# jtdaugherty/flux

Measured on AMD Instinct MI355X. Metric: Msamples/sec on demo2.yml (fixed spp), higher is better.
Workload: dtype f64

## Files before the change

### flux_amd/csrc/abi.hip

```cpp
#include <hip/hip_runtime.h>

#include <chrono>
#include <cmath>
#include <cstdarg>
#include <cstdio>
#include <cstring>
#include <memory>
#include <new>
#include <algorithm>
#include <cstdlib>
#include <string>
#include <vector>

#include "../../include/flux_abi.h"
#include "flux_device.h"
#include "flux_tables.h"
#include "flux_math_coeffs.h"

#include "flux_ctx.h"

namespace flux {

thread_local std::string g_last_error;

// ... 42 lines not shown
    hipError_t e = hipMemcpy(d, xy, sizeof(xy), hipMemcpyHostToDevice);
    if (e == hipSuccess) e = flux::generate_sampler_grid(FLUX_SAMPLER_REGULAR, 0, 2, d, nullptr, nullptr);
    if (e == hipSuccess) e = hipStreamCreateWithFlags(&s, hipStreamNonBlocking);
    if (s) (void)hipStreamDestroy(s);
    (void)hipFree(d);
    if (e != hipSuccess) return fail(FLUX_E_DEVICE, "flux_device_warmup: %s", hipGetErrorString(e));
    return FLUX_OK;
}

static void free_ctx(flux_ctx *c) {
    if (!c) return;
    DeviceGuard g(c->device);
    if (c->ev0) (void)hipEventDestroy(c->ev0);
    if (c->ev1) (void)hipEventDestroy(c->ev1);
    (void)hipFree(c->d_shapes);
    (void)hipFree(c->d_mats);
    (void)hipFree(c->d_fscene);
    (void)hipFree(c->d_pix);
    (void)hipFree(c->d_disc);
    (void)hipFree(c->d_hemi);
    (void)hipFree(c->d_gloss);
    (void)hipFree(c->d_glossx);
    (void)hipFree(c->d_gxoff);
    (void)hipFree(c->d_setrows);
    (void)hipFree(c->d_rowperm);
    (void)hipFree(c->d_invperm);
    (void)hipFree(c->d_stats);
    (void)hipFree(c->d_tris);
    (void)hipFree(c->d_nodes);
    (void)hipFree(c->d_nodesq);
    (void)hipFree(c->d_arena);
    (void)hipFree(c->d_out);
    delete c;
}

void flux_ctx_destroy(flux_ctx *ctx) { free_ctx(ctx); }

}

namespace flux {

static int validate_material(const flux_material &m, const char *what, uint64_t i) {
    if (m.kind < FLUX_MAT_MATTE || m.kind > FLUX_MAT_DIELECTRIC)
        return fail(FLUX_E_INVALID, "%s %llu: unknown material kind %d", what, (unsigned long long)i, m.kind);
    if (m.kind == FLUX_MAT_DIELECTRIC && !(std::isfinite(m.k) && m.k > 0.0))
        return fail(FLUX_E_INVALID, "%s %llu: dielectric refraction index must be finite and > 0, got %g", what, (unsigned long long)i, m.k);
// ... 103 lines not shown
    };
    auto copy = [&](void *dst, const auto &v) {
        if (e == hipSuccess) e = hipMemcpy(dst, v.data(), v.size() * sizeof(v[0]), hipMemcpyHostToDevice);
    };
    auto alloc_copy = [&](auto **p, const auto &v) {
        alloc(p, v.size() * sizeof(v[0]));
        copy(*p, v);
    };
    alloc_copy(&c->d_shapes, h.shapes);
    alloc(&c->d_mats, h.mats.size() * sizeof(DevMaterial) + h.wtab.size() * sizeof(double));
    copy(c->d_mats, h.mats);
    copy(c->d_mats + h.mats.size(), h.wtab);
    alloc_copy(&c->d_fscene, h.fscene);
    alloc(&c->d_pix, pix_bytes);
    alloc(&c->d_disc, pix_bytes);
    alloc(&c->d_hemi, hemi_bytes);
    alloc(&c->d_gloss, pix_bytes * 2);
    const char *tables_env = std::getenv("FLUX_SAMPLE_TABLES");
    const int gx_stride = (tables_env && std::atoi(tables_env) == 0) ? 0 : h.rp.gx_stride;
    if (gx_stride) {
        alloc(&c->d_glossx, own * c->N * (size_t)gx_stride);
        alloc_copy(&c->d_gxoff, h.gx_off);
    }
    alloc(&c->d_setrows, own * sizeof(DevSetRows));
    alloc(&c->d_rowperm, perm_bytes);
    alloc(&c->d_invperm, perm_bytes);
    alloc(&c->d_stats, FLUX_NUM_STATS * sizeof(unsigned long long));
    if (!h.tris.empty()) {
        alloc_copy(&c->d_tris, h.tris);
        alloc_copy(&c->d_nodes, h.nodes);
        alloc_copy(&c->d_nodesq, h.nodesq);
        if (!h.arena.empty()) alloc_copy(&c->d_arena, h.arena);
    }
    if (e == hipSuccess) e = hipMemset(c->d_stats, 0, FLUX_NUM_STATS * sizeof(unsigned long long));
    laps.lap(FLUX_CREATE_MS_UPLOAD);
    if (e == hipSuccess) e = hipEventCreate(&c->ev0);
    if (e == hipSuccess) e = hipEventCreate(&c->ev1);
    laps.lap(FLUX_CREATE_MS_OTHER);
    double tab_ms[3] = {0, 0, 0};
    if (e == hipSuccess)
        e = generate_tables(seed, c->S, c->sets, c->D, c->n, c->H, c->d_pix, c->d_disc, c->d_hemi, c->d_rowperm, c->d_invperm, nullptr, tab_ms);
    if (e == hipSuccess) {
        e = generate_gloss_table(c->d_pix, (size_t)c->sets.count * c->N, c->d_gloss, nullptr);
        if (e == hipSuccess && gx_stride)
            e = generate_glossx_table(c->d_gloss, (size_t)c->sets.count * c->N, h.gx_inv_e1.data(), h.rp.n_gloss_exp, gx_stride / 16,
                                      c->d_glossx, nullptr);
// ... 11 lines not shown
            rows[m].hemi = c->d_hemi + m * c->D * c->N * kHemiDoubles;
            rows[m].gloss = c->d_gloss + m * c->N * 4;
            rows[m].glossx = gx_stride ? c->d_glossx + m * c->N * (size_t)(gx_stride / 16) : nullptr;
        }
        copy(c->d_setrows, rows);
    }
    if (e != hipSuccess)
        return fail(e == hipErrorOutOfMemory ? FLUX_E_NOMEM : FLUX_E_DEVICE, "flux_ctx_create: %s", hipGetErrorString(e));

    RenderParams &rp = c->rp;
    rp = h.rp;
    rp.pixel_denom = 1.0 / (double)((uint64_t)c->n * c->n);
    rp.max_depth = (int32_t)c->D;
    rp.nsamp = c->N;
    rp.shapes = c->d_shapes;
    rp.mats = c->d_mats;
    rp.pix = c->d_pix;
    rp.disc = c->d_disc;
    rp.hemi = c->d_hemi;
    rp.gloss = c->d_gloss;
    rp.glossx = c->d_glossx;
    rp.gx_off = c->d_gxoff;
    rp.gx_stride = gx_stride;
    rp.set_rows = c->d_setrows;
    rp.rowperm = c->d_rowperm;
    rp.invperm = c->d_invperm;
    for (int k = 0; k < 12; k++) rp.exp2c[k] = fastmath::kExp2Poly[k];
    rp.tris = c->d_tris;
    rp.nodes = c->d_nodes;
    rp.nodesq = c->d_nodesq;
    rp.nodes4 = reinterpret_cast<const DevNode4Q *>(c->d_arena);
    const unsigned char *fs = c->d_fscene;
    rp.fsph = reinterpret_cast<const DevScanSphere *>(fs + h.fs.sph);
    rp.fpln = reinterpret_cast<const DevScanPlane *>(fs + h.fs.pln);
    rp.frec = reinterpret_cast<const DevHitRec *>(fs + h.fs.rec);
    rp.fsph32 = h.filter32 ? reinterpret_cast<const DevScanSphere32 *>(fs + h.fs.s32) : nullptr;
    rp.f32_half = rp.fsph32 && h.f32_half >= 0 ? rp.fsph32 + h.f32_half : nullptr;
    rp.f32_top = rp.fsph32 ? rp.fsph32 + h.f32_top : nullptr;
    rp.sshapes = reinterpret_cast<const DevShape *>(fs + h.fs.ss);
    rp.pxc = reinterpret_cast<const double *>(fs + h.fs.pxc);
    rp.fdsk = reinterpret_cast<const DevScanDisk *>(fs + h.fs.dsk);
    rp.fbox = reinterpret_cast<const DevScanBox *>(fs + h.fs.box);
    laps.lap(FLUX_CREATE_MS_UPLOAD);
    laps.ms[FLUX_CREATE_MS_TOTAL] = 0.0;
    for (int k = 1; k < FLUX_CREATE_TIMING_WORDS; k++) laps.ms[FLUX_CREATE_MS_TOTAL] += laps.ms[k];
    for (int k = 0; k < FLUX_CREATE_TIMING_WORDS; k++) c->create_ms[k] = laps.ms[k];
// ... 454 lines not shown
```

### flux_amd/csrc/flux_ctx.h

```cpp
#pragma once
#include <hip/hip_runtime.h>

#include <chrono>
#include <new>
#include <string>
#include <system_error>

#include "../../include/flux_abi.h"
#include "flux_device.h"
#include "flux_tables.h"
#include "scene_build.h"

namespace flux {

extern thread_local std::string g_last_error;
int fail(int code, const char *fmt, ...) __attribute__((format(printf, 2, 3)));

template <class F> int no_throw(F &&f) {
    try {
        return f();
    } catch (const std::bad_alloc &) {
        return fail(FLUX_E_NOMEM, "host allocation failed");
    } catch (const std::system_error &e) {
        return fail(FLUX_E_NOMEM, "%s", e.what());
// ... 31 lines not shown

#define HIP_TRY(expr)                                                                             \
    do {                                                                                          \
        hipError_t e_ = (expr);                                                                   \
        if (e_ != hipSuccess)                                                                     \
            return flux::fail(e_ == hipErrorOutOfMemory ? FLUX_E_NOMEM : FLUX_E_DEVICE, "%s: %s", \
                              #expr, hipGetErrorString(e_));                                      \
    } while (0)

struct flux_ctx {
    int device = 0;
    flux::RenderParams rp{};
    uint64_t seed = 0;
    uint32_t n = 0, N = 0, D = 0, S = 0, W = 0, H = 0;
    flux::SetRange sets{0, 1, 0};
    flux::DevShape *d_shapes = nullptr;
    flux::DevMaterial *d_mats = nullptr;
    unsigned char *d_fscene = nullptr;
    double2 *d_pix = nullptr, *d_disc = nullptr;
    double *d_hemi = nullptr;
    double *d_gloss = nullptr;
    double2 *d_glossx = nullptr;
    int32_t *d_gxoff = nullptr;
    flux::DevSetRows *d_setrows = nullptr;
    int32_t *d_rowperm = nullptr, *d_invperm = nullptr;
    unsigned long long *d_stats = nullptr;
    bool stats_on = false;
    flux::DevTri *d_tris = nullptr;
    flux::DevNode *d_nodes = nullptr;
    flux::DevNode4A *d_arena = nullptr;
    flux::DevNodeQ *d_nodesq = nullptr;
    flux::BvhInfo bvh{};
    int traversal = FLUX_TRAVERSE_BVH;
    int variant = FLUX_KERNEL_DEFAULT;
    int math = FLUX_MATH_FAST;
    double *d_out = nullptr;
    size_t d_out_doubles = 0;
    hipEvent_t ev0 = nullptr, ev1 = nullptr;
    bool timed = false;
    uint64_t device_bytes = 0;
    double U[3], V[3], Wv[3];
    double create_ms[FLUX_CREATE_TIMING_WORDS] = {};
};
```

### flux_amd/csrc/flux_device.h

```cpp
#pragma once
#include <hip/hip_runtime.h>
#include <stdint.h>

#include "flux_bvh.h"


#ifndef FLUX_UNI_SPHERES
#define FLUX_UNI_SPHERES 2
#endif
#ifndef FLUX_BVH_WIDE_MAX_STACK
#define FLUX_BVH_WIDE_MAX_STACK 48
#endif
#ifndef FLUX_MAX_WAVES_PER_PIXEL
#define FLUX_MAX_WAVES_PER_PIXEL 4
#endif
#ifndef FLUX_MIN_SAMPLES_PER_WAVE
#define FLUX_MIN_SAMPLES_PER_WAVE 4096
#endif

namespace flux {

constexpr int kHemiDoubles = 4;
constexpr double kTMin = 0.0005;
constexpr double kPi = 3.14159265358979323846264338327950288;
// ... 138 lines not shown
    int32_t self_skip;
    int32_t n_uni, uni_idx[2];
    int32_t unit_dirs;
    int32_t env_short, pad_env;
    double env_radius;
    double t_min, env_deep;
    double env_px, env_py, env_pz, env_rr;
    double env_eps;
    const DevScanSphere32 *f32_half, *f32_top;
    int32_t f32_groups;
    uint32_t f32_valid;
    double fwx, fwy, fwz;
    const double *pxc;
    const DevSetRows *set_rows;
    double exp2c[12];
    const DevScanDisk *fdsk;
    int32_t n_dsk;
    int32_t has_diel;
    const double2 *glossx;
    const int32_t *gx_off;
    int32_t gx_stride, n_gloss_exp;
    const DevScanBox *fbox;
    int32_t n_box;
};

__host__ __device__ inline int hit_records(const RenderParams &p) { return p.n_sph + p.n_pln + p.n_dsk + 6 * p.n_box; }

}
```

### flux_amd/csrc/flux_plan.h

```cpp
#pragma once
#include <stddef.h>
#include <stdint.h>

#include "flux_device.h"

#ifndef FLUX_BLOCK_THREADS
#define FLUX_BLOCK_THREADS 64
#endif
#ifndef FLUX_WPE_SPLIT
#define FLUX_WPE_SPLIT 5
#endif
#ifndef FLUX_HITQ_MIN_TAKE
#define FLUX_HITQ_MIN_TAKE 32
#endif

namespace flux {

constexpr int kGlossExpSlots = 4;

constexpr int kQueueDoubles = 9;
constexpr int kQueueBytesPerWave = (kQueueDoubles * 64) * 8 + 2 * 64 * 4;
constexpr int kHitQDoubles = 7;
constexpr int kHitQInts = 3;
constexpr int kHitQBytesPerSlot = kHitQDoubles * 8 + kHitQInts * 4;
constexpr uint32_t kHitQDwordsPerSlot = kHitQBytesPerSlot / 4;
constexpr uint32_t hitq_entry_dword(uint32_t C, uint32_t k) { return (C - 1u - k) * kHitQDwordsPerSlot; }
constexpr bool hitq_admits_phase_a(uint32_t C, uint32_t nhit) { return nhit + 64u <= C; }

enum KernelCopy { kCopyStrict = 0, kCopyFast = 1, kCopyFastDiel = 2 };
KernelCopy kernel_copy(const RenderParams &p, int math);

struct LaunchPlan {
    int kernel = -1;
    unsigned block = 64;
    uint64_t blocks = 0;
    size_t lds = 0;
    unsigned waves_per_pixel = 1;
    int lds_scene = 0;
    int hq_cap = 0, hq_th = 0, hq_bits = 0;
    int copy = kCopyFast;
    int tris = 0;
    int typ = 0;
    int max32 = 0;
};
LaunchPlan plan_render(const RenderParams &p, int variant, int math);

size_t lane_stacks_lds(int math, size_t depth, bool tris, size_t bvh_stack, size_t lanes);
size_t shade_rays_lds(const RenderParams &p, int math);

}
// ... 1 lines not shown
```

### flux_amd/csrc/launch_plan.cpp

```cpp
#include <algorithm>
#include <cstdlib>

#include "flux_plan.h"
#include "../../include/flux_abi.h"

namespace flux {

KernelCopy kernel_copy(const RenderParams &p, int math) {
    if (math == FLUX_MATH_STRICT) return kCopyStrict;
    return p.has_diel ? kCopyFastDiel : kCopyFast;
}

size_t lane_stacks_lds(int math, size_t depth, bool tris, size_t bvh_stack, size_t lanes) {
    return (math == FLUX_MATH_STRICT ? depth * 4 * lanes * sizeof(double) : 0) + (tris ? bvh_stack * lanes * sizeof(int) : 0);
}

size_t shade_rays_lds(const RenderParams &p, int math) {
    return lane_stacks_lds(math, (size_t)p.max_depth, p.n_tris > 0, (size_t)p.bvh_stack, 64);
}

static bool split_typ(const RenderParams &p) {
    return p.n_sph <= 32 && p.glossy_long == 0 && p.unit_dirs == 1 && p.self_skip == 1 && p.env_short == 1 && p.n_uni == 1 &&
           p.fsph32 != nullptr && p.n_dsk == 0 && p.n_box == 0 && p.has_diel == 0 && (p.n_gloss_exp == 0 || p.gx_stride != 0);
}
static bool bvh4_typ(const RenderParams &p, bool lds_scene) {
    return lds_scene && p.n_sph <= 32 && p.glossy_long == 0 && p.unit_dirs == 1 && p.self_skip == 1 && p.n_uni == 1 &&
           p.fsph32 != nullptr && p.n_dsk == 0 && p.n_box == 0 && p.has_diel == 0;
}

LaunchPlan plan_render(const RenderParams &p, int variant, int math) {
    LaunchPlan L;
    L.copy = kernel_copy(p, math);
    const bool fast = L.copy != kCopyStrict;
    const uint32_t N = p.nsamp;
    const uint64_t npix = (uint64_t)p.num_rows * (uint64_t)p.img_w;
    if (npix == 0 || p.set_count <= 0) return L;
    if (variant == FLUX_KERNEL_DEFAULT) variant = N >= 256u ? FLUX_KERNEL_SPLIT : FLUX_KERNEL_REFILL;
    if (N < 64u) variant = FLUX_KERNEL_STATIC;
    const uint32_t lpp = N >= 64u ? 64u : N;
    const uint32_t ppw = 64u / lpp;
    uint64_t waves = (npix + ppw - 1) / ppw;
    if (variant != FLUX_KERNEL_STATIC && p.num_sets == (uint32_t)p.img_w)
        waves = 8ull * ((uint64_t)(p.set_count / 8) * (uint64_t)p.num_rows +
                        ((uint64_t)(p.set_count % 8) * (uint64_t)p.num_rows + 7u) / 8u);
    unsigned K = 1;
    if (variant != FLUX_KERNEL_STATIC)
        while (K * 2u <= (unsigned)FLUX_MAX_WAVES_PER_PIXEL && (uint64_t)K * 2u * FLUX_MIN_SAMPLES_PER_WAVE <= N) K *= 2u;
    const bool tris = p.n_tris > 0;
    if (!fast && variant != FLUX_KERNEL_STATIC)
        while (K > 1u && lane_stacks_lds(math, (size_t)p.max_depth, tris, (size_t)p.bvh_stack, 64 * K) > 60 * 1024) K /= 2u;
    const unsigned block = (variant == FLUX_KERNEL_STATIC) ? FLUX_BLOCK_THREADS : 64u * K;
    const unsigned wpb = (variant == FLUX_KERNEL_STATIC) ? block / 64 : 1u;
    L.blocks = (waves + wpb - 1) / wpb;
    if (fast && variant != FLUX_KERNEL_STATIC && tris && p.bvh_stack > 0) {
        L.block = 64;
        size_t lds4 = (size_t)(p.bvh4_stack > 0 ? p.bvh4_stack : 1) * 64 * sizeof(int);
        const size_t scene4 = (size_t)hit_records(p) * sizeof(DevHitRec) + (size_t)p.n_mats * sizeof(DevMaterial) +
                              (size_t)p.n_sph * sizeof(DevScanSphere);
        const bool lds_scene4 = lds4 + scene4 <= 7680;
        if (lds_scene4) lds4 += scene4;
        if (p.nodes4 != nullptr && p.bvh4_stack <= FLUX_BVH_WIDE_MAX_STACK) {
            L.kernel = 4;
            L.lds = lds4;
            L.lds_scene = lds_scene4 ? 1 : 0;
            L.typ = bvh4_typ(p, lds_scene4) ? 1 : 0;
        } else {
            L.kernel = 3;
            L.lds = (size_t)p.bvh_stack * 64 * sizeof(int);
        }
        return L;
    }
    const size_t scene_lds = (size_t)hit_records(p) * sizeof(DevHitRec) + (size_t)p.n_sph * sizeof(DevScanSphere);
    if (fast && variant == FLUX_KERNEL_SPLIT && !tris && p.n_sph <= 64 && scene_lds <= 16384) {
        L.kernel = 2;
        L.block = block;
        L.waves_per_pixel = K;
        L.lds = (size_t)kQueueBytesPerWave * K + scene_lds;
        L.typ = split_typ(p) ? 1 : 0;
        L.max32 = p.n_sph <= 32 ? 1 : 0;
        if (p.glossy_long == 0 && p.has_diel == 0) {
            const size_t granules = (size_t)128 * K / (4 * FLUX_WPE_SPLIT);
            const size_t per_wave = granules * 1280 > scene_lds + 96 ? (granules * 1280 - scene_lds - 96) / K : 0;
            uint32_t cap = (uint32_t)(per_wave / kHitQBytesPerSlot) & ~1u;
            if (const char *e = std::getenv("FLUX_SPLIT_HITQ_CAP")) cap = std::min(cap, (uint32_t)std::max(0, std::atoi(e)) & ~1u);
            uint32_t th = cap > 64u + FLUX_HITQ_MIN_TAKE ? std::min(64u, cap - 64u) : FLUX_HITQ_MIN_TAKE;
            if (const char *e = std::getenv("FLUX_SPLIT_HITQ_TAKE_AT")) th = (uint32_t)std::max(1, std::min(64, std::atoi(e)));
            int bits = 1;
            while ((1 << bits) < hit_records(p)) ++bits;
            if (cap >= 64u + th && bits * p.max_depth <= 32) {
                L.hq_cap = (int)cap;
                L.hq_th = (int)th;
                L.hq_bits = bits;
                L.lds = (size_t)cap * kHitQBytesPerSlot * K + scene_lds;
            }
        }
        return L;
    }
    L.kernel = variant == FLUX_KERNEL_STATIC ? 0 : 1;
    L.block = block;
    L.waves_per_pixel = variant == FLUX_KERNEL_STATIC ? 1 : K;
    L.lds = lane_stacks_lds(math, (size_t)p.max_depth, tris, (size_t)p.bvh_stack, block);
    L.tris = tris ? 1 : 0;
    return L;
}

}
```

### flux_amd/csrc/render_body.inc

```

#undef FLUX_STAGE
#if FLUX_FAST
#define FLUX_STAGE() __builtin_amdgcn_sched_barrier(0)
#else
#define FLUX_STAGE() ((void)0)
#endif

struct Ray {
    double ox, oy, oz, dx, dy, dz;
};

typedef const __attribute__((address_space(4))) RenderParams *ParamsInKernarg;
static_assert(sizeof(DevMaterial) % 16 == 0, "the bounce-weight records behind the materials are read as double2");
__device__ __forceinline__ const RenderParams &relaunder_params(uint32_t tick) {
    ParamsInKernarg p = (ParamsInKernarg)__builtin_amdgcn_kernarg_segment_ptr();
    asm("" : "+s"(p) : "s"(tick));
    return *(const RenderParams *)p;
}

__device__ __forceinline__ unsigned long long ballot64(bool b) { return __builtin_amdgcn_ballot_w64(b); }
__device__ __forceinline__ bool any64(bool b) { return __builtin_amdgcn_ballot_w64(b) != 0ull; }
__device__ __forceinline__ bool all64(bool b) { return __builtin_amdgcn_ballot_w64(!b) == 0ull; }

typedef double flux_d2 __attribute__((ext_vector_type(2)));
// ... 1607 lines not shown
            const double e = fastmath::fsqrt_nonneg(__builtin_fmax(dq, 0.0));
            double t = (-hb - e) * rs;
            if (!(t > tmin)) t = (-hb + e) * rs;
            bool ok = dq >= 0.0 && t > tmin;
            if (any_zflat) {
                if (zflat && box_z_nan_miss(P, r, k)) ok = false;
            }
            if (ok) {
                bool take = best < 0 || t < tb;
                if (!take && t == tb) take = best >= P.n_sph ? P.frec[k].orig_id < best_id : k < best;
                if (take) {
                    best = k;
                    tb = t;
                }
            }
        }
    }
}

__device__ __forceinline__ double lds_dword_pair(const uint32_t *p) { return __hiloint2double((int)p[1], (int)p[0]); }
__device__ __forceinline__ void lds_dword_pair_store(uint32_t *p, double v) {
    p[0] = (uint32_t)__double2loint(v);
    p[1] = (uint32_t)__double2hiint(v);
}

template <bool STATS, bool MAX32, bool TYP, bool HQ = false>
__global__ __launch_bounds__(64 * FLUX_MAX_WAVES_PER_PIXEL, FLUX_WPE_SPLIT) void render_split_kernel(const RenderParams P0, int hq_cap, int hq_th,
                                                                                                  int hq_bits) {
    (void)hq_cap;
    (void)hq_th;
    (void)hq_bits;
    const RenderParams &P = P0;
    extern __shared__ double lds_stack[];
    __shared__ double part[FLUX_MAX_WAVES_PER_PIXEL][3];
    const int tid = threadIdx.x;
    const uint32_t lane = tid & 63;
    const uint32_t N = P.nsamp;
    const uint32_t K = blockDim.x >> 6, sub = (uint32_t)__builtin_amdgcn_readfirstlane(tid >> 6);
    const uint32_t s_lo = (uint32_t)((uint64_t)N * sub / K), s_hi = (uint32_t)((uint64_t)N * (sub + 1) / K);
    const int n_rec = TYP ? P.n_sph + P.n_pln + P.n_dsk : hit_records(P);
    const size_t scene_lds_bytes = (size_t)n_rec * sizeof(DevHitRec) + (size_t)P.n_sph * sizeof(DevScanSphere);
    double *q = lds_stack + scene_lds_bytes / 8 + (size_t)sub * (HQ ? (size_t)hq_cap * kHitQBytesPerSlot / 8 : kQueueBytesPerWave / 8);
    int *qi = reinterpret_cast<int *>(q + (size_t)kQueueDoubles * 64);
    const char *const frec_lds = reinterpret_cast<const char *>(lds_stack);
    const char *const fsph_lds = frec_lds + (size_t)n_rec * sizeof(DevHitRec);
    {
// ... 74 lines not shown
                        Lr = Lg = Lb = 0.0;
                        if (STATS) st.c[7]++;
                    }
                    if (!cont) {
                        fold_path(p, nullptr, 0, Lr, Lg, Lb);
                        sr += Lr;
                        sg += Lg;
                        sb += Lb;
                    }
                }
                i = ia;
                ml = (uint32_t)hit;
                if (!cont) p.depth = kDeadDepth;
            }
            if (nhit) {
                const unsigned long long freemask = ballot64(p.depth == kDeadDepth);
                const uint32_t nfree = (uint32_t)__popcll(freemask);
                const uint32_t take = nfree < nhit ? nfree : nhit;
                if (!run_a || take >= H || !(next < s_hi && hitq_admits_phase_a(C, nhit))) {
                    const uint32_t rank = __builtin_amdgcn_mbcnt_hi((uint32_t)(freemask >> 32),
                                                                    __builtin_amdgcn_mbcnt_lo((uint32_t)freemask, 0u));
                    if (p.depth == kDeadDepth && rank < take) {
                        FLUX_CENSUS(P, 15);
                        const uint32_t *e = pool + hitq_entry_dword(C, nhit - 1u - rank);
                        p.r.ox = lds_dword_pair(e + 3);
                        p.r.oy = lds_dword_pair(e + 5);
                        p.r.oz = lds_dword_pair(e + 7);
                        p.r.dx = lds_dword_pair(e + 9);
                        p.r.dy = lds_dword_pair(e + 11);
                        p.r.dz = lds_dword_pair(e + 13);
                        const double t = lds_dword_pair(e + 15);
                        const int hd = (int)e[0];
                        i = e[1];
                        const int hit = hd & 0xffff;
                        p.depth = hd >> 16;
                        ml = e[2];
                        const DevHitRec &R0 = recs[ml & bmask];
                        p.tr = R0.fr;
                        p.tg = R0.fg;
                        p.tb = R0.fb;
                        for (int k = 1; k < p.depth - 1; ++k) {
                            const DevHitRec &Rk = recs[(ml >> (k * hq_bits)) & bmask];
                            p.tr *= Rk.fr;
                            p.tg *= Rk.fg;
                            p.tb *= Rk.fb;
                        }
                        ml |= (uint32_t)hit << ((p.depth - 1) * hq_bits);
                        bounce_parked_hit<STATS, TYP>(P, p, set_p, i, hit, t, st, 6, frec_lds);
                    }
                    nhit -= take;
                }
            }
            if (__builtin_expect((nhit | (s_hi - next)) == 0u, 0)) {
                if (!any64(p.depth != kDeadDepth)) break;
            }
            FLUX_TRIP(P, 10);
            const bool live = p.depth != kDeadDepth;
            const bool trace = p.depth <= P.max_depth;
            double Lr = 0.0, Lg = 0.0, Lb = 0.0;
            bool cont = false;
            int hit = -1;
            double t = 0.0;
            if (trace) {
                FLUX_CENSUS(P, 3);
                if (STATS) st.c[1]++;
                const float ofx = (float)p.r.ox, ofy = (float)p.r.oy, ofz = (float)p.r.oz;
                const float oo32 = __builtin_fmaf(ofz, ofz, __builtin_fmaf(ofy, ofy, ofx * ofx));
                if (__builtin_expect((ballot64(p.r.dz == 0.0) | ballot64(!(oo32 < 0.999e6f))) != 0ull, 0))
                    scan_shapes_fast<true, true, MAX32, TYP, 1>(P, p.r, p.self, hit, t, nullptr, fsph_lds);
                else
                    scan_shapes_fast<true, true, MAX32, TYP, 0>(P, p.r, p.self, hit, t, nullptr, fsph_lds);
                cont = shade_hit_fast<STATS, false, true, TYP, false, false>(P, p, set_p, i, hit, -1, t, Lr, Lg, Lb, st, 0, frec_lds);
            }
            if (live && !cont) {
                if (STATS && !trace) st.c[7]++;
                fold_path(p, nullptr, 0, Lr, Lg, Lb);
                sr += Lr;
                sg += Lg;
                sb += Lb;
            }
            const unsigned long long pmask = ballot64(cont);
            if (cont) {
                uint32_t *e = pool + hitq_entry_dword(C, nhit + __builtin_amdgcn_mbcnt_hi((uint32_t)(pmask >> 32),
                                                                                           __builtin_amdgcn_mbcnt_lo((uint32_t)pmask, 0u)));
                e[0] = (uint32_t)(hit | (p.depth << 16));
                e[1] = i;
                e[2] = ml;
                lds_dword_pair_store(e + 3, p.r.ox);
                lds_dword_pair_store(e + 5, p.r.oy);
                lds_dword_pair_store(e + 7, p.r.oz);
                lds_dword_pair_store(e + 9, p.r.dx);
                lds_dword_pair_store(e + 11, p.r.dy);
                lds_dword_pair_store(e + 13, p.r.dz);
                lds_dword_pair_store(e + 15, t);
            }
            nhit += (uint32_t)__popcll(pmask);
        }
    }
    if (!HQ && wave_on) {
        unsigned long long cand_mask, in_mask;
        double in_t0;
        pixel_sphere_mask(P, row, col, lane, cand_mask, in_mask, in_t0);

#ifdef FLUX_DEBUG_CLOCK
        long long lap_store[8] = {0, 0, 0, 0, 0, 0, 0, (long long)__builtin_readcyclecounter()};
        long long *lap = lap_store;
#else
        long long *lap = nullptr;
#endif
        uint32_t next = s_lo;
        uint32_t qcount = 0;
        uint32_t i = 0;
        constexpr int kDeadDepth = 0x7fffffff;
        Path p;
        path_begin(p);
        p.depth = kDeadDepth;
        p.sq = make_double2(0.0, 0.0);
// ... 827 lines not shown
        else render_bvh_kernel<false><<<g, b, lds, stream>>>(p);
        return hipGetLastError();
    }
    if (L.kernel == 4) {
        if (L.typ) {
#if FLUX_DIEL
            return hipErrorInvalidValue;
#else
            if (stats) render_bvh4_kernel<true, true, true><<<g, b, lds, stream>>>(p);
            else render_bvh4_kernel<false, true, true><<<g, b, lds, stream>>>(p);
#endif
        } else if (L.lds_scene) {
            if (stats) render_bvh4_kernel<true, true, false><<<g, b, lds, stream>>>(p);
            else render_bvh4_kernel<false, true, false><<<g, b, lds, stream>>>(p);
        } else {
            if (stats) render_bvh4_kernel<true, false, false><<<g, b, lds, stream>>>(p);
            else render_bvh4_kernel<false, false, false><<<g, b, lds, stream>>>(p);
        }
        return hipGetLastError();
    }
    if (L.kernel == 2) {
        const int c = L.hq_cap, h = L.hq_th, bits = L.hq_bits;
        const bool hq = L.hq_cap > 0;
#define FLUX_LAUNCH_SPLIT(MAX32, TYP, HQ)                                                                      \
    do {                                                                                                       \
        if (stats) render_split_kernel<true, MAX32, TYP, HQ><<<g, b, lds, stream>>>(p, c, h, bits);            \
        else render_split_kernel<false, MAX32, TYP, HQ><<<g, b, lds, stream>>>(p, c, h, bits);                 \
    } while (0)
#if FLUX_DIEL
        if (L.typ || hq) return hipErrorInvalidValue;
#else
        if (L.typ) {
            if (hq) FLUX_LAUNCH_SPLIT(true, true, true);
            else FLUX_LAUNCH_SPLIT(true, true, false);
            return hipGetLastError();
        }
        if (hq) {
            if (L.max32) FLUX_LAUNCH_SPLIT(true, false, true);
            else FLUX_LAUNCH_SPLIT(false, false, true);
            return hipGetLastError();
        }
#endif
        if (L.max32) FLUX_LAUNCH_SPLIT(true, false, false);
        else FLUX_LAUNCH_SPLIT(false, false, false);
#undef FLUX_LAUNCH_SPLIT
        return hipGetLastError();
    }
#endif
    if (L.kernel == 0)
        FLUX_LAUNCH(render_static_kernel);
// ... 6 lines not shown
```

### flux_amd/csrc/scene_build.cpp

```cpp
#include "scene_build.h"

#include <algorithm>
#include <cmath>
#include <cstdio>
#include <cstdlib>
#include <cstring>

#include "joining_thread.h"

namespace flux {

namespace {

void normalize3(const double in[3], double out[3]) {
    double len = std::sqrt(in[0] * in[0] + in[1] * in[1] + in[2] * in[2]);
    out[0] = in[0] / len;
    out[1] = in[1] / len;
    out[2] = in[2] / len;
}
void cross3(const double a[3], const double b[3], double o[3]) {
    o[0] = a[1] * b[2] - a[2] * b[1];
    o[1] = a[2] * b[0] - a[0] * b[2];
    o[2] = a[0] * b[1] - a[1] * b[0];
}
// ... 216 lines not shown
    }
    rp.t_min = kTMin;
    rp.env_deep = -(4.0 * kTMin) * rp.env_radius;
    rp.env_eps = 1e-9;
    if (rp.n_uni == 1) {
        const DevScanSphere &es = fsph[rp.uni_idx[0]];
        rp.env_px = es.px; rp.env_py = es.py; rp.env_pz = es.pz; rp.env_rr = es.rr;
    }
    rp.f32_valid = fsph.size() >= 32 ? 0xffffffffu : (1u << fsph.size()) - 1u;
    if (h.filter32 && fsph.size() <= 32) {
        int pairs = ((int)fsph.size() + 1) >> 1;
        const int rem = pairs & 3;
        if (rem == 1 || rem == 2) {
            h.f32_half = pairs - rem;
            pairs -= rem;
        } else if (rem == 3) {
            pairs += 1;
        }
        rp.f32_groups = pairs / 4;
        h.f32_top = pairs;
    }
}

int build_meshes(const flux_scene_desc &scene, HostScene &h, std::string &error) {
    const size_t ns = (size_t)scene.num_shapes;
    std::vector<size_t> first((size_t)scene.num_meshes + 1, 0);
    for (size_t m = 0; m < (size_t)scene.num_meshes; m++) first[m + 1] = first[m] + (size_t)scene.meshes[m].num_triangles;
    if ((uint64_t)first.back() * sizeof(DevTri) >= (1ull << 32)) {
        char buf[160];
        std::snprintf(buf, sizeof(buf), "%zu triangles exceed the %llu a context can hold", first.back(),
                      (unsigned long long)((1ull << 32) / sizeof(DevTri)));
        error = buf;
        return FLUX_E_INVALID;
    }
    h.tris.assign(first.back(), DevTri{});
    auto make = [&](size_t lo, size_t hi) {
        size_t m = 0;
        for (size_t g = lo; g < hi; g++) {
            while (g >= first[m + 1]) m++;
            const flux_mesh &me = scene.meshes[m];
            const size_t k = g - first[m];
            const double *a = me.vertices + 3 * (size_t)me.indices[3 * k];
            const double *b = me.vertices + 3 * (size_t)me.indices[3 * k + 1];
            const double *d = me.vertices + 3 * (size_t)me.indices[3 * k + 2];
            DevTri &t = h.tris[g];
            t.v0x = a[0]; t.v0y = a[1]; t.v0z = a[2];
// ... 136 lines not shown
```

### flux_amd/csrc/scene_build.h

```cpp
#pragma once
#include <cstddef>
#include <string>
#include <vector>

#include "../../include/flux_abi.h"
#include "flux_device.h"
#include "flux_plan.h"

namespace flux {

struct FsceneLayout {
    size_t sph = 0;
    size_t pln = 0;
    size_t rec = 0;
    size_t s32 = 0;
    size_t ss = 0;
    size_t pxc = 0;
    size_t dsk = 0;
    size_t box = 0;
    size_t bytes = 0;
};
FsceneLayout fscene_layout(size_t n_sph, size_t n_pln, size_t n_dsk, size_t n_box, size_t n_shapes, uint32_t W, uint32_t H);

struct HostScene {
    std::vector<DevShape> shapes;
    std::vector<DevMaterial> mats;
    std::vector<double> wtab;
    FsceneLayout fs;
    std::vector<unsigned char> fscene;
    std::vector<DevTri> tris;
    std::vector<DevNode> nodes;
    std::vector<DevNodeQ> nodesq;
    std::vector<DevNode4A> arena;
    BvhInfo bvh;
    double U[3] = {}, V[3] = {}, W[3] = {};
    RenderParams rp{};
    bool filter32 = false;
    int f32_half = -1;
    int f32_top = 0;
    std::vector<double> gx_inv_e1;
    std::vector<int32_t> gx_off;
};

int build_host_scene(const flux_scene_desc &scene, HostScene &out, std::string &error);

}
```

Before: 51240.

## Precompute path throughput products in a global table indexed by hit-record list

Builds a host-side table of per-channel throughput products for every possible sequence of hit records up to max depth, uploads it, and has the split kernel fetch the parked ray's throughput with three global loads. This replaces the per-resumed-ray loop of LDS record reads and f64 multiplies. It also reorders the hit-queue slot layout so doubles come first and uses a 24-bit multiply for the slot address. In exchange it adds up to 4 MiB of device memory, global-load latency on the resume path, and host build time at context creation.

```diff
diff --git a/flux_amd/csrc/abi.hip b/flux_amd/csrc/abi.hip
--- a/flux_amd/csrc/abi.hip
+++ b/flux_amd/csrc/abi.hip
@@ -88,6 +88,7 @@
     (void)hipFree(c->d_gloss);
     (void)hipFree(c->d_glossx);
     (void)hipFree(c->d_gxoff);
+    (void)hipFree(c->d_tput);
     (void)hipFree(c->d_setrows);
     (void)hipFree(c->d_rowperm);
     (void)hipFree(c->d_invperm);
@@ -237,6 +238,18 @@
         alloc(&c->d_glossx, own * c->N * (size_t)gx_stride);
         alloc_copy(&c->d_gxoff, h.gx_off);
     }
+    int tput_bits = 0;
+    {
+        RenderParams job = h.rp;
+        job.nsamp = c->N;
+        job.max_depth = (int32_t)c->D;
+        const char *tput_env = std::getenv("FLUX_THROUGHPUT_TABLE");
+        if (!(tput_env && std::atoi(tput_env) == 0) && tput_table_bytes(job, &tput_bits)) {
+            std::vector<double> tput;
+            build_tput_table(h, tput_bits, (int)c->D, tput);
+            alloc_copy(&c->d_tput, tput);
+        }
+    }
     alloc(&c->d_setrows, own * sizeof(DevSetRows));
     alloc(&c->d_rowperm, perm_bytes);
     alloc(&c->d_invperm, perm_bytes);
@@ -294,6 +307,8 @@
     rp.glossx = c->d_glossx;
     rp.gx_off = c->d_gxoff;
     rp.gx_stride = gx_stride;
+    rp.tput = c->d_tput;
+    rp.tput_bits = c->d_tput ? tput_bits : 0;
     rp.set_rows = c->d_setrows;
     rp.rowperm = c->d_rowperm;
     rp.invperm = c->d_invperm;
diff --git a/flux_amd/csrc/flux_ctx.h b/flux_amd/csrc/flux_ctx.h
--- a/flux_amd/csrc/flux_ctx.h
+++ b/flux_amd/csrc/flux_ctx.h
@@ -77,6 +77,7 @@
     double *d_gloss = nullptr;
     double2 *d_glossx = nullptr;
     int32_t *d_gxoff = nullptr;
+    double *d_tput = nullptr;
     flux::DevSetRows *d_setrows = nullptr;
     int32_t *d_rowperm = nullptr, *d_invperm = nullptr;
     unsigned long long *d_stats = nullptr;
diff --git a/flux_amd/csrc/flux_device.h b/flux_amd/csrc/flux_device.h
--- a/flux_amd/csrc/flux_device.h
+++ b/flux_amd/csrc/flux_device.h
@@ -184,6 +184,8 @@
     int32_t gx_stride, n_gloss_exp;
     const DevScanBox *fbox;
     int32_t n_box;
+    int32_t tput_bits;
+    const double *tput;
 };
 
 __host__ __device__ inline int hit_records(const RenderParams &p) { return p.n_sph + p.n_pln + p.n_dsk + 6 * p.n_box; }
diff --git a/flux_amd/csrc/flux_plan.h b/flux_amd/csrc/flux_plan.h
--- a/flux_amd/csrc/flux_plan.h
+++ b/flux_amd/csrc/flux_plan.h
@@ -23,9 +23,20 @@
 constexpr int kHitQDoubles = 7;
 constexpr int kHitQInts = 3;
 constexpr int kHitQBytesPerSlot = kHitQDoubles * 8 + kHitQInts * 4;
+enum HitQField : uint32_t {
+    kHitQOx = 0, kHitQOy = 2, kHitQOz = 4, kHitQDx = 6, kHitQDy = 8, kHitQDz = 10, kHitQT = 12,
+    kHitQHitDepth = 14,
+    kHitQSample = 15,
+    kHitQList = 16,
+};
 constexpr uint32_t kHitQDwordsPerSlot = kHitQBytesPerSlot / 4;
 constexpr uint32_t hitq_entry_dword(uint32_t C, uint32_t k) { return (C - 1u - k) * kHitQDwordsPerSlot; }
 constexpr bool hitq_admits_phase_a(uint32_t C, uint32_t nhit) { return nhit + 64u <= C; }
+
+constexpr size_t kTputEntryBytes = 24;
+constexpr size_t kTputTableMaxBytes = (size_t)4 << 20;
+constexpr uint32_t tput_index(uint32_t list_bits, uint32_t ml) { return (1u << list_bits) | ml; }
+size_t tput_table_bytes(const RenderParams &p, int *bits = nullptr);
 
 enum KernelCopy { kCopyStrict = 0, kCopyFast = 1, kCopyFastDiel = 2 };
 KernelCopy kernel_copy(const RenderParams &p, int math);
diff --git a/flux_amd/csrc/launch_plan.cpp b/flux_amd/csrc/launch_plan.cpp
--- a/flux_amd/csrc/launch_plan.cpp
+++ b/flux_amd/csrc/launch_plan.cpp
@@ -28,6 +28,43 @@
            p.fsph32 != nullptr && p.n_dsk == 0 && p.n_box == 0 && p.has_diel == 0;
 }
 
+static unsigned waves_per_pixel(uint32_t N) {
+    unsigned K = 1;
+    while (K * 2u <= (unsigned)FLUX_MAX_WAVES_PER_PIXEL && (uint64_t)K * 2u * FLUX_MIN_SAMPLES_PER_WAVE <= N) K *= 2u;
+    return K;
+}
+
+static size_t split_scene_lds(const RenderParams &p) {
+    return (size_t)hit_records(p) * sizeof(DevHitRec) + (size_t)p.n_sph * sizeof(DevScanSphere);
+}
+static bool split_serves(const RenderParams &p) { return p.n_tris == 0 && p.n_sph <= 64 && split_scene_lds(p) <= 16384; }
+
+static bool plan_hitq(const RenderParams &p, unsigned K, size_t scene_lds, uint32_t &cap, uint32_t &th, int &bits) {
+    if (p.glossy_long != 0 || p.has_diel != 0) return false;
+    const size_t granules = (size_t)128 * K / (4 * FLUX_WPE_SPLIT);
+    const size_t per_wave = granules * 1280 > scene_lds + 96 ? (granules * 1280 - scene_lds - 96) / K : 0;
+    cap = (uint32_t)(per_wave / kHitQBytesPerSlot) & ~1u;
+    if (const char *e = std::getenv("FLUX_SPLIT_HITQ_CAP")) cap = std::min(cap, (uint32_t)std::max(0, std::atoi(e)) & ~1u);
+    th = cap > 64u + FLUX_HITQ_MIN_TAKE ? std::min(64u, cap - 64u) : FLUX_HITQ_MIN_TAKE;
+    if (const char *e = std::getenv("FLUX_SPLIT_HITQ_TAKE_AT")) th = (uint32_t)std::max(1, std::min(64, std::atoi(e)));
+    bits = 1;
+    while ((1 << bits) < hit_records(p)) ++bits;
+    return cap >= 64u + th && bits * p.max_depth <= 32;
+}
+
+size_t tput_table_bytes(const RenderParams &p, int *bits_out) {
+    uint32_t cap, th;
+    int bits;
+    if (p.nsamp < 64u || p.max_depth < 2 || !split_serves(p) || !plan_hitq(p, waves_per_pixel(p.nsamp), split_scene_lds(p), cap, th, bits))
+        return 0;
+    const int list_bits = bits * (p.max_depth - 1);
+    if (list_bits + 1 > 24) return 0;
+    const size_t bytes = ((size_t)2 << list_bits) * kTputEntryBytes;
+    if (bytes > kTputTableMaxBytes) return 0;
+    if (bits_out) *bits_out = bits;
+    return bytes;
+}
+
 LaunchPlan plan_render(const RenderParams &p, int variant, int math) {
     LaunchPlan L;
     L.copy = kernel_copy(p, math);
@@ -43,9 +80,7 @@
     if (variant != FLUX_KERNEL_STATIC && p.num_sets == (uint32_t)p.img_w)
         waves = 8ull * ((uint64_t)(p.set_count / 8) * (uint64_t)p.num_rows +
                         ((uint64_t)(p.set_count % 8) * (uint64_t)p.num_rows + 7u) / 8u);
-    unsigned K = 1;
-    if (variant != FLUX_KERNEL_STATIC)
-        while (K * 2u <= (unsigned)FLUX_MAX_WAVES_PER_PIXEL && (uint64_t)K * 2u * FLUX_MIN_SAMPLES_PER_WAVE <= N) K *= 2u;
+    unsigned K = variant != FLUX_KERNEL_STATIC ? waves_per_pixel(N) : 1u;
     const bool tris = p.n_tris > 0;
     if (!fast && variant != FLUX_KERNEL_STATIC)
         while (K > 1u && lane_stacks_lds(math, (size_t)p.max_depth, tris, (size_t)p.bvh_stack, 64 * K) > 60 * 1024) K /= 2u;
@@ -70,29 +105,21 @@
         }
         return L;
     }
-    const size_t scene_lds = (size_t)hit_records(p) * sizeof(DevHitRec) + (size_t)p.n_sph * sizeof(DevScanSphere);
-    if (fast && variant == FLUX_KERNEL_SPLIT && !tris && p.n_sph <= 64 && scene_lds <= 16384) {
+    const size_t scene_lds = split_scene_lds(p);
+    if (fast && variant == FLUX_KERNEL_SPLIT && split_serves(p)) {
         L.kernel = 2;
         L.block = block;
         L.waves_per_pixel = K;
         L.lds = (size_t)kQueueBytesPerWave * K + scene_lds;
         L.typ = split_typ(p) ? 1 : 0;
         L.max32 = p.n_sph <= 32 ? 1 : 0;
-        if (p.glossy_long == 0 && p.has_diel == 0) {
-            const size_t granules = (size_t)128 * K / (4 * FLUX_WPE_SPLIT);
-            const size_t per_wave = granules * 1280 > scene_lds + 96 ? (granules * 1280 - scene_lds - 96) / K : 0;
-            uint32_t cap = (uint32_t)(per_wave / kHitQBytesPerSlot) & ~1u;
-            if (const char *e = std::getenv("FLUX_SPLIT_HITQ_CAP")) cap = std::min(cap, (uint32_t)std::max(0, std::atoi(e)) & ~1u);
-            uint32_t th = cap > 64u + FLUX_HITQ_MIN_TAKE ? std::min(64u, cap - 64u) : FLUX_HITQ_MIN_TAKE;
-            if (const char *e = std::getenv("FLUX_SPLIT_HITQ_TAKE_AT")) th = (uint32_t)std::max(1, std::min(64, std::atoi(e)));
-            int bits = 1;
-            while ((1 << bits) < hit_records(p)) ++bits;
-            if (cap >= 64u + th && bits * p.max_depth <= 32) {
-                L.hq_cap = (int)cap;
-                L.hq_th = (int)th;
-                L.hq_bits = bits;
-                L.lds = (size_t)cap * kHitQBytesPerSlot * K + scene_lds;
-            }
+        uint32_t cap, th;
+        int bits;
+        if (plan_hitq(p, K, scene_lds, cap, th, bits)) {
+            L.hq_cap = (int)cap;
+            L.hq_th = (int)th;
+            L.hq_bits = bits;
+            L.lds = (size_t)cap * kHitQBytesPerSlot * K + scene_lds;
         }
         return L;
     }
diff --git a/flux_amd/csrc/render_body.inc b/flux_amd/csrc/render_body.inc
--- a/flux_amd/csrc/render_body.inc
+++ b/flux_amd/csrc/render_body.inc
@@ -1653,6 +1653,10 @@
 __device__ __forceinline__ void lds_dword_pair_store(uint32_t *p, double v) {
     p[0] = (uint32_t)__double2loint(v);
     p[1] = (uint32_t)__double2hiint(v);
+}
+
+__device__ __forceinline__ uint32_t *hitq_entry(uint32_t *pool, uint32_t C, uint32_t k) {
+    return reinterpret_cast<uint32_t *>(reinterpret_cast<char *>(pool) + __umul24(C - 1u - k, (uint32_t)kHitQBytesPerSlot));
 }
 
 template <bool STATS, bool MAX32, bool TYP, bool HQ = false>
@@ -1773,30 +1777,39 @@
                                                                     __builtin_amdgcn_mbcnt_lo((uint32_t)freemask, 0u));
                     if (p.depth == kDeadDepth && rank < take) {
                         FLUX_CENSUS(P, 15);
-                        const uint32_t *e = pool + hitq_entry_dword(C, nhit - 1u - rank);
-                        p.r.ox = lds_dword_pair(e + 3);
-                        p.r.oy = lds_dword_pair(e + 5);
-                        p.r.oz = lds_dword_pair(e + 7);
-                        p.r.dx = lds_dword_pair(e + 9);
-                        p.r.dy = lds_dword_pair(e + 11);
-                        p.r.dz = lds_dword_pair(e + 13);
-                        const double t = lds_dword_pair(e + 15);
-                        const int hd = (int)e[0];
-                        i = e[1];
+                        const uint32_t *e = hitq_entry(pool, C, nhit - 1u - rank);
+                        p.r.ox = lds_dword_pair(e + kHitQOx);
+                        p.r.oy = lds_dword_pair(e + kHitQOy);
+                        p.r.oz = lds_dword_pair(e + kHitQOz);
+                        p.r.dx = lds_dword_pair(e + kHitQDx);
+                        p.r.dy = lds_dword_pair(e + kHitQDy);
+                        p.r.dz = lds_dword_pair(e + kHitQDz);
+                        const double t = lds_dword_pair(e + kHitQT);
+                        const int hd = (int)e[kHitQHitDepth];
+                        i = e[kHitQSample];
                         const int hit = hd & 0xffff;
                         p.depth = hd >> 16;
-                        ml = e[2];
-                        const DevHitRec &R0 = recs[ml & bmask];
-                        p.tr = R0.fr;
-                        p.tg = R0.fg;
-                        p.tb = R0.fb;
-                        for (int k = 1; k < p.depth - 1; ++k) {
-                            const DevHitRec &Rk = recs[(ml >> (k * hq_bits)) & bmask];
-                            p.tr *= Rk.fr;
-                            p.tg *= Rk.fg;
-                            p.tb *= Rk.fb;
+                        ml = e[kHitQList];
+                        const uint32_t list_bits = __umul24((uint32_t)(p.depth - 1), (uint32_t)hq_bits);
+                        if (P.tput != nullptr) {
+                            const uint32_t off = __umul24(tput_index(list_bits, ml), (uint32_t)kTputEntryBytes);
+                            p.tr = gather_global<double>(P.tput, off);
+                            p.tg = gather_global<double>(P.tput, off + 8u);
+                            p.tb = gather_global<double>(P.tput, off + 16u);
+                        } else {
+                            const DevHitRec &R0 = recs[ml & bmask];
+                            p.tr = R0.fr;
+                            p.tg = R0.fg;
+                            p.tb = R0.fb;
+#pragma unroll 1
+                            for (int k = 1; k < p.depth - 1; ++k) {
+                                const DevHitRec &Rk = recs[(ml >> (k * hq_bits)) & bmask];
+                                p.tr *= Rk.fr;
+                                p.tg *= Rk.fg;
+                                p.tb *= Rk.fb;
+                            }
                         }
-                        ml |= (uint32_t)hit << ((p.depth - 1) * hq_bits);
+                        ml |= (uint32_t)hit << list_bits;
                         bounce_parked_hit<STATS, TYP>(P, p, set_p, i, hit, t, st, 6, frec_lds);
                     }
                     nhit -= take;
@@ -1832,18 +1845,18 @@
             }
             const unsigned long long pmask = ballot64(cont);
             if (cont) {
-                uint32_t *e = pool + hitq_entry_dword(C, nhit + __builtin_amdgcn_mbcnt_hi((uint32_t)(pmask >> 32),
-                                                                                           __builtin_amdgcn_mbcnt_lo((uint32_t)pmask, 0u)));
-                e[0] = (uint32_t)(hit | (p.depth << 16));
-                e[1] = i;
-                e[2] = ml;
-                lds_dword_pair_store(e + 3, p.r.ox);
-                lds_dword_pair_store(e + 5, p.r.oy);
-                lds_dword_pair_store(e + 7, p.r.oz);
-                lds_dword_pair_store(e + 9, p.r.dx);
-                lds_dword_pair_store(e + 11, p.r.dy);
-                lds_dword_pair_store(e + 13, p.r.dz);
-                lds_dword_pair_store(e + 15, t);
+                uint32_t *e = hitq_entry(pool, C, nhit + __builtin_amdgcn_mbcnt_hi((uint32_t)(pmask >> 32),
+                                                                                   __builtin_amdgcn_mbcnt_lo((uint32_t)pmask, 0u)));
+                lds_dword_pair_store(e + kHitQOx, p.r.ox);
+                lds_dword_pair_store(e + kHitQOy, p.r.oy);
+                lds_dword_pair_store(e + kHitQOz, p.r.oz);
+                lds_dword_pair_store(e + kHitQDx, p.r.dx);
+                lds_dword_pair_store(e + kHitQDy, p.r.dy);
+                lds_dword_pair_store(e + kHitQDz, p.r.dz);
+                lds_dword_pair_store(e + kHitQT, t);
+                e[kHitQHitDepth] = (uint32_t)(hit | (p.depth << 16));
+                e[kHitQSample] = i;
+                e[kHitQList] = ml;
             }
             nhit += (uint32_t)__popcll(pmask);
         }
@@ -2717,10 +2730,12 @@
     if (L.kernel == 2) {
         const int c = L.hq_cap, h = L.hq_th, bits = L.hq_bits;
         const bool hq = L.hq_cap > 0;
+        RenderParams ps = p;
+        if (!hq || ps.tput_bits != bits) ps.tput = nullptr;
 #define FLUX_LAUNCH_SPLIT(MAX32, TYP, HQ)                                                                      \
     do {                                                                                                       \
-        if (stats) render_split_kernel<true, MAX32, TYP, HQ><<<g, b, lds, stream>>>(p, c, h, bits);            \
-        else render_split_kernel<false, MAX32, TYP, HQ><<<g, b, lds, stream>>>(p, c, h, bits);                 \
+        if (stats) render_split_kernel<true, MAX32, TYP, HQ><<<g, b, lds, stream>>>(ps, c, h, bits);           \
+        else render_split_kernel<false, MAX32, TYP, HQ><<<g, b, lds, stream>>>(ps, c, h, bits);                \
     } while (0)
 #if FLUX_DIEL
         if (L.typ || hq) return hipErrorInvalidValue;
diff --git a/flux_amd/csrc/scene_build.cpp b/flux_amd/csrc/scene_build.cpp
--- a/flux_amd/csrc/scene_build.cpp
+++ b/flux_amd/csrc/scene_build.cpp
@@ -262,6 +262,35 @@
     }
 }
 
+}
+
+void build_tput_table(const HostScene &h, int bits, int max_depth, std::vector<double> &out) {
+    const DevHitRec *rec = reinterpret_cast<const DevHitRec *>(h.fscene.data() + h.fs.rec);
+    const uint32_t n_rec = (uint32_t)hit_records(h.rp);
+    out.assign(((size_t)2 << (bits * (max_depth - 1))) * 3, 0.0);
+    for (uint32_t e = 0; e < n_rec; e++) {
+        double *t = &out[(size_t)tput_index((uint32_t)bits, e) * 3];
+        t[0] = rec[e].fr; t[1] = rec[e].fg; t[2] = rec[e].fb;
+    }
+    std::vector<uint32_t> heads(n_rec), lists;
+    for (uint32_t e = 0; e < n_rec; e++) heads[e] = e;
+    for (int n = 2; n < max_depth; n++) {
+        const uint32_t head_bits = (uint32_t)(bits * (n - 1));
+        lists.clear();
+        lists.reserve(heads.size() * n_rec);
+        for (uint32_t e = 0; e < n_rec; e++)
+            for (const uint32_t head : heads) {
+                const uint32_t ml = head | (e << head_bits);
+                const double *a = &out[(size_t)tput_index(head_bits, head) * 3];
+                double *t = &out[(size_t)tput_index(head_bits + (uint32_t)bits, ml) * 3];
+                t[0] = a[0] * rec[e].fr; t[1] = a[1] * rec[e].fg; t[2] = a[2] * rec[e].fb;
+                lists.push_back(ml);
+            }
+        heads.swap(lists);
+    }
+}
+
+namespace {
 int build_meshes(const flux_scene_desc &scene, HostScene &h, std::string &error) {
     const size_t ns = (size_t)scene.num_shapes;
     std::vector<size_t> first((size_t)scene.num_meshes + 1, 0);
diff --git a/flux_amd/csrc/scene_build.h b/flux_amd/csrc/scene_build.h
--- a/flux_amd/csrc/scene_build.h
+++ b/flux_amd/csrc/scene_build.h
@@ -44,4 +44,6 @@
 
 int build_host_scene(const flux_scene_desc &scene, HostScene &out, std::string &error);
 
+void build_tput_table(const HostScene &h, int bits, int max_depth, std::vector<double> &out);
+
 }
diff --git a/profiles/r10_throughput_table/take_block_after.s b/profiles/r10_throughput_table/take_block_after.s
--- /dev/null
+++ b/profiles/r10_throughput_table/take_block_after.s
@@ -0,0 +1,78 @@
+	s_and_b64 s[2:3], s[2:3], vcc
+	s_and_saveexec_b64 s[8:9], s[2:3]
+	s_cbranch_execz .LBB24_159
+	s_sub_i32 s2, s28, s46
+	v_add_u32_e32 v0, s2, v0
+	s_movk_i32 s2, 0x44
+	v_mov_b32_e32 v1, s76
+	v_mad_u32_u24 v0, v0, s2, v1
+	ds_read2_b32 v[50:51], v0 offset0:8 offset1:9
+	ds_read2_b32 v[52:53], v0 offset0:10 offset1:11
+	ds_read2_b32 v[48:49], v0 offset0:12 offset1:13
+	ds_read2_b32 v[44:45], v0 offset0:14 offset1:15
+	ds_read2_b32 v[38:39], v0 offset1:1
+	ds_read2_b32 v[40:41], v0 offset0:2 offset1:3
+	ds_read2_b32 v[42:43], v0 offset0:4 offset1:5
+	ds_read2_b32 v[54:55], v0 offset0:6 offset1:7
+	s_load_dwordx2 s[4:5], s[68:69], 0x300
+	ds_read_b32 v77, v0 offset:64
+	v_mov_b32_e32 v0, -1
+	s_waitcnt lgkmcnt(0)
+	v_add_u32_sdwa v0, sext(v44), v0 dst_sel:DWORD dst_unused:UNUSED_PAD src0_sel:WORD_1 src1_sel:DWORD
+	v_mul_u32_u24_e32 v78, s83, v0
+	s_cmp_eq_u64 s[4:5], 0
+	s_mov_b64 s[2:3], 0
+	s_cbranch_scc1 .LBB24_137
+	v_lshl_or_b32 v0, 1, v78, v77
+	v_mul_u32_u24_e32 v4, 24, v0
+	global_load_dwordx2 v[46:47], v4, s[4:5] offset:16
+	global_load_dwordx4 v[0:3], v4, s[4:5]
+	s_andn2_b64 vcc, exec, s[2:3]
+	s_cbranch_vccz .LBB24_138
+	s_branch .LBB24_143
+.LBB24_133:
+	s_or_b64 exec, exec, s[12:13]
+.LBB24_137:
+.LBB24_138:
+	s_waitcnt vmcnt(0)
+	v_and_b32_e32 v0, s77, v77
+	s_movk_i32 s2, 0x60
+	v_mul_lo_u32 v0, v0, s2
+	v_add_u32_e32 v4, 0x60, v0
+	ds_read2_b64 v[0:3], v4 offset0:4 offset1:5
+	ds_read_b64 v[46:47], v4 offset:48
+	v_mov_b32_e32 v4, 2
+	v_cmp_gt_i32_sdwa s[4:5], sext(v44), v4 src0_sel:WORD_1 src1_sel:DWORD
+	s_and_saveexec_b64 s[2:3], s[4:5]
+	s_cbranch_execz .LBB24_142
+	v_mov_b32_e32 v4, -2
+	v_add_u32_sdwa v4, sext(v44), v4 dst_sel:DWORD dst_unused:UNUSED_PAD src0_sel:WORD_1 src1_sel:DWORD
+	s_mov_b64 s[4:5], 0
+	s_mov_b32 s6, s30
+.LBB24_140:
+	v_lshrrev_b32_e32 v5, s6, v77
+	s_movk_i32 s7, 0x60
+	v_and_b32_e32 v5, s77, v5
+	v_mul_lo_u32 v5, v5, s7
+	v_add_u32_e32 v5, 0x60, v5
+	ds_read2_b64 v[6:9], v5 offset0:4 offset1:5
+	ds_read_b64 v[10:11], v5 offset:48
+	v_add_u32_e32 v4, -1, v4
+	s_add_i32 s6, s6, s30
+	v_cmp_eq_u32_e32 vcc, 0, v4
+	s_or_b64 s[4:5], vcc, s[4:5]
+	s_waitcnt lgkmcnt(1)
+	v_mul_f64 v[0:1], v[0:1], v[6:7]
+	v_mul_f64 v[2:3], v[2:3], v[8:9]
+	s_waitcnt lgkmcnt(0)
+	v_mul_f64 v[46:47], v[46:47], v[10:11]
+	s_andn2_b64 exec, exec, s[4:5]
+	s_cbranch_execnz .LBB24_140
+	s_or_b64 exec, exec, s[4:5]
+.LBB24_142:
+	s_or_b64 exec, exec, s[2:3]
+.LBB24_143:
+	v_and_b32_e32 v79, 0xffff, v44
+	s_movk_i32 s2, 0x60
+	v_mov_b32_e32 v4, 0x60
+	v_mad_u32_u24 v16, v79, s2, v4
diff --git a/profiles/r10_throughput_table/take_block_before.s b/profiles/r10_throughput_table/take_block_before.s
--- /dev/null
+++ b/profiles/r10_throughput_table/take_block_before.s
@@ -0,0 +1,183 @@
+	s_sub_i32 s2, s28, s46
+	v_add_u32_e32 v0, s2, v0
+	s_movk_i32 s2, 0x44
+	v_mul_lo_u32 v0, v0, s2
+	v_add_u32_e32 v0, s76, v0
+	ds_read2_b32 v[38:39], v0 offset0:2 offset1:3
+	ds_read2_b32 v[8:9], v0 offset0:8 offset1:9
+	ds_read2_b32 v[10:11], v0 offset0:10 offset1:11
+	ds_read2_b32 v[4:5], v0 offset0:12 offset1:13
+	ds_read2_b32 v[6:7], v0 offset0:14 offset1:15
+	ds_read2_b32 v[12:13], v0 offset0:4 offset1:5
+	ds_read2_b32 v[14:15], v0 offset0:6 offset1:7
+	ds_read2_b32 v[44:45], v0 offset1:1
+	s_waitcnt lgkmcnt(7)
+	v_and_b32_e32 v1, s77, v38
+	s_movk_i32 s2, 0x60
+	v_mul_lo_u32 v1, v1, s2
+	v_add_u32_e32 v16, 0x60, v1
+	ds_read_b32 v41, v0 offset:64
+	ds_read2_b64 v[0:3], v16 offset0:4 offset1:5
+	ds_read_b64 v[46:47], v16 offset:48
+	v_mov_b32_e32 v16, 2
+	s_waitcnt lgkmcnt(3)
+	v_cmp_gt_i32_sdwa s[4:5], sext(v44), v16 src0_sel:WORD_1 src1_sel:DWORD
+	s_and_saveexec_b64 s[2:3], s[4:5]
+	s_cbranch_execz .LBB24_141
+	v_mov_b32_e32 v17, -3
+	v_mov_b32_e32 v16, -2
+	v_add_u32_sdwa v17, sext(v44), v17 dst_sel:DWORD dst_unused:UNUSED_PAD src0_sel:WORD_1 src1_sel:DWORD
+	v_add_u32_sdwa v16, sext(v44), v16 dst_sel:DWORD dst_unused:UNUSED_PAD src0_sel:WORD_1 src1_sel:DWORD
+	v_cmp_lt_u32_e32 vcc, 6, v17
+	v_mov_b32_e32 v18, 1
+	s_and_saveexec_b64 s[4:5], vcc
+	s_cbranch_execz .LBB24_136
+	v_and_b32_e32 v17, -8, v16
+	s_mov_b32 s10, 0
+	s_mov_b64 s[6:7], 0
+	s_mov_b32 s11, 0
+.LBB24_134:
+	s_add_i32 s13, s30, s10
+	s_add_i32 s15, s83, s10
+	s_add_i32 s16, s85, s10
+	s_add_i32 s17, s86, s10
+	s_add_i32 s18, s87, s10
+	s_add_i32 s19, s88, s10
+	s_add_i32 s20, s89, s10
+	s_add_i32 s10, s84, s10
+	v_lshrrev_b32_e32 v19, s13, v38
+	v_lshrrev_b32_e32 v20, s15, v38
+	v_lshrrev_b32_e32 v21, s16, v38
+	v_lshrrev_b32_e32 v22, s17, v38
+	v_lshrrev_b32_e32 v23, s18, v38
+	v_lshrrev_b32_e32 v24, s19, v38
+	v_lshrrev_b32_e32 v25, s20, v38
+	s_movk_i32 s14, 0x60
+	v_lshrrev_b32_e32 v40, s10, v38
+	v_and_b32_e32 v19, s77, v19
+	v_and_b32_e32 v20, s77, v20
+	v_and_b32_e32 v21, s77, v21
+	v_and_b32_e32 v22, s77, v22
+	v_and_b32_e32 v23, s77, v23
+	v_and_b32_e32 v24, s77, v24
+	v_and_b32_e32 v25, s77, v25
+	v_and_b32_e32 v40, s77, v40
+	v_mul_lo_u32 v19, v19, s14
+	v_mul_lo_u32 v20, v20, s14
+	v_mul_lo_u32 v21, v21, s14
+	v_mul_lo_u32 v22, v22, s14
+	v_mul_lo_u32 v23, v23, s14
+	v_mul_lo_u32 v24, v24, s14
+	v_mul_lo_u32 v25, v25, s14
+	v_mul_lo_u32 v40, v40, s14
+	v_add_u32_e32 v19, 0x60, v19
+	v_add_u32_e32 v42, 0x60, v20
+	v_add_u32_e32 v56, 0x60, v21
+	v_add_u32_e32 v60, 0x60, v22
+	v_add_u32_e32 v64, 0x60, v23
+	v_add_u32_e32 v68, 0x60, v24
+	v_add_u32_e32 v72, 0x60, v25
+	v_add_u32_e32 v40, 0x60, v40
+	ds_read2_b64 v[20:23], v19 offset0:4 offset1:5
+	ds_read_b64 v[24:25], v19 offset:48
+	ds_read2_b64 v[48:51], v42 offset0:4 offset1:5
+	ds_read_b64 v[42:43], v42 offset:48
+	ds_read2_b64 v[52:55], v56 offset0:4 offset1:5
+	ds_read_b64 v[76:77], v56 offset:48
+	ds_read2_b64 v[56:59], v60 offset0:4 offset1:5
+	ds_read_b64 v[80:81], v60 offset:48
+	ds_read2_b64 v[60:63], v64 offset0:4 offset1:5
+	ds_read_b64 v[82:83], v64 offset:48
+	ds_read2_b64 v[64:67], v68 offset0:4 offset1:5
+	ds_read_b64 v[84:85], v68 offset:48
+	ds_read2_b64 v[68:71], v72 offset0:4 offset1:5
+	ds_read_b64 v[86:87], v72 offset:48
+	ds_read2_b64 v[72:75], v40 offset0:4 offset1:5
+	ds_read_b64 v[88:89], v40 offset:48
+	s_waitcnt lgkmcnt(14)
+	v_mul_f64 v[0:1], v[0:1], v[20:21]
+	v_mul_f64 v[2:3], v[2:3], v[22:23]
+	v_mul_f64 v[20:21], v[46:47], v[24:25]
+	s_waitcnt lgkmcnt(13)
+	v_mul_f64 v[0:1], v[0:1], v[48:49]
+	v_mul_f64 v[2:3], v[2:3], v[50:51]
+	s_waitcnt lgkmcnt(12)
+	v_mul_f64 v[20:21], v[20:21], v[42:43]
+	s_waitcnt lgkmcnt(11)
+	v_mul_f64 v[0:1], v[0:1], v[52:53]
+	v_mul_f64 v[2:3], v[2:3], v[54:55]
+	s_waitcnt lgkmcnt(10)
+	v_mul_f64 v[20:21], v[20:21], v[76:77]
+	s_waitcnt lgkmcnt(9)
+	v_mul_f64 v[0:1], v[0:1], v[56:57]
+	v_mul_f64 v[2:3], v[2:3], v[58:59]
+	s_waitcnt lgkmcnt(8)
+	v_mul_f64 v[20:21], v[20:21], v[80:81]
+	s_waitcnt lgkmcnt(7)
+	v_mul_f64 v[0:1], v[0:1], v[60:61]
+	v_mul_f64 v[2:3], v[2:3], v[62:63]
+	s_waitcnt lgkmcnt(6)
+	v_mul_f64 v[20:21], v[20:21], v[82:83]
+	s_add_i32 s21, s11, 8
+	s_waitcnt lgkmcnt(5)
+	v_mul_f64 v[0:1], v[0:1], v[64:65]
+	v_mul_f64 v[2:3], v[2:3], v[66:67]
+	s_waitcnt lgkmcnt(4)
+	v_mul_f64 v[20:21], v[20:21], v[84:85]
+	s_add_i32 s11, s11, 9
+	v_cmp_eq_u32_e32 vcc, s21, v17
+	s_waitcnt lgkmcnt(3)
+	v_mul_f64 v[0:1], v[0:1], v[68:69]
+	v_mul_f64 v[2:3], v[2:3], v[70:71]
+	s_waitcnt lgkmcnt(2)
+	v_mul_f64 v[20:21], v[20:21], v[86:87]
+	v_mov_b32_e32 v18, s11
+	s_mov_b32 s11, s21
+	s_or_b64 s[6:7], vcc, s[6:7]
+	s_waitcnt lgkmcnt(1)
+	v_mul_f64 v[0:1], v[0:1], v[72:73]
+	v_mul_f64 v[2:3], v[2:3], v[74:75]
+	s_waitcnt lgkmcnt(0)
+	v_mul_f64 v[46:47], v[20:21], v[88:89]
+	s_andn2_b64 exec, exec, s[6:7]
+	s_cbranch_execnz .LBB24_134
+	s_or_b64 exec, exec, s[6:7]
+.LBB24_136:
+	s_or_b64 exec, exec, s[4:5]
+	v_and_b32_e32 v16, 7, v16
+	v_cmp_ne_u32_e32 vcc, 0, v16
+	s_and_saveexec_b64 s[4:5], vcc
+	s_cbranch_execz .LBB24_140
+	v_mul_lo_u32 v17, s30, v18
+	s_mov_b64 s[6:7], 0
+.LBB24_138:
+	v_lshrrev_b32_e32 v18, v17, v38
+	s_movk_i32 s10, 0x60
+	v_and_b32_e32 v18, s77, v18
+	v_mul_lo_u32 v18, v18, s10
+	v_add_u32_e32 v22, 0x60, v18
+	ds_read2_b64 v[18:21], v22 offset0:4 offset1:5
+	ds_read_b64 v[22:23], v22 offset:48
+	v_add_u32_e32 v16, -1, v16
+	v_cmp_eq_u32_e32 vcc, 0, v16
+	v_add_u32_e32 v17, s30, v17
+	s_or_b64 s[6:7], vcc, s[6:7]
+	s_waitcnt lgkmcnt(1)
+	v_mul_f64 v[0:1], v[0:1], v[18:19]
+	v_mul_f64 v[2:3], v[2:3], v[20:21]
+	s_waitcnt lgkmcnt(0)
+	v_mul_f64 v[46:47], v[46:47], v[22:23]
+	s_andn2_b64 exec, exec, s[6:7]
+	s_cbranch_execnz .LBB24_138
+	s_or_b64 exec, exec, s[6:7]
+.LBB24_140:
+	s_or_b64 exec, exec, s[4:5]
+.LBB24_141:
+	s_or_b64 exec, exec, s[2:3]
+	v_pk_mov_b32 v[42:43], v[38:39], v[12:13] op_sel:[1,0]
+	v_pk_mov_b32 v[60:61], v[10:11], v[4:5] op_sel:[1,0]
+	v_pk_mov_b32 v[62:63], v[4:5], v[6:7] op_sel:[1,0]
+	v_and_b32_e32 v39, 0xffff, v44
+	s_movk_i32 s2, 0x60
+	v_mov_b32_e32 v4, 0x60
+	v_mad_u32_u24 v16, v39, s2, v4
```

After: 52580, median of 6. 2.6% higher.
